# Soltanilara/av-aloha

Measured on AMD Instinct MI355X. Metric: env-steps/sec (whole node) at 4096 parallel envs, SlotInsertion-3Arms, higher is better.
Workload: dtype f32

## Files before the change

### av_aloha_amd/_ffi.py

```python
import ctypes as C
import os

import numpy as np

HERE = os.path.dirname(os.path.abspath(__file__))
LIB_PATH = os.path.join(HERE, "libavsim.so")

AVSIM_IO_DEVICE = 1
AVSIM_F64_PHYSICS = 2
IK_REFERENCE, IK_DLS = 0, 1
NDIMS = 12

_lib = None


class AvsimError(RuntimeError):
    pass


def lib():
    global _lib
    if _lib is None:
        if not os.path.exists(LIB_PATH):
            raise AvsimError(f"{LIB_PATH} is missing: build it with `python -m av_aloha_amd.build` "
                             "(there is no CPU fallback for the simulation path)")
        L = C.CDLL(LIB_PATH)
        vp, i32, u32, dbl = C.c_void_p, C.c_int, C.c_uint32, C.c_double
        L.avsim_create.argtypes = [vp, C.c_size_t, i32, i32, u32, C.POINTER(vp)]
        L.avsim_destroy.argtypes = [vp]
        L.avsim_destroy.restype = None
        L.avsim_last_error.argtypes = [vp]
        L.avsim_last_error.restype = C.c_char_p
        L.avsim_dims.argtypes = [vp, vp]
        L.avsim_set_option.argtypes = [vp, C.c_char_p, dbl]
        L.avsim_reset.argtypes = [vp, vp, vp]
        L.avsim_step.argtypes = [vp, vp, i32, vp, vp, vp]
        L.avsim_step_cartesian.argtypes = [vp, vp, i32, i32, vp, vp, vp]
        L.avsim_step_ctrl.argtypes = [vp, i32, vp, vp, vp]
        L.avsim_ik.argtypes = [vp, i32, i32, i32, i32, vp, vp, vp, vp]
        L.avsim_fk_jac.argtypes = [vp, i32, i32, vp, vp, vp]
        L.avsim_observe.argtypes = [vp, vp, vp, vp]
        L.avsim_set_qpos.argtypes = [vp, vp]
        L.avsim_get_state.argtypes = [vp, vp, vp, vp, vp]
        L.avsim_set_state.argtypes = [vp, vp, vp, vp, vp]
        L.avsim_get_reset_poses.argtypes = [vp, vp]
        L.avsim_set_reset_poses.argtypes = [vp, vp]
        L.avsim_get_latch.argtypes = [vp, vp]
        L.avsim_set_latch.argtypes = [vp, vp]
        L.avsim_get_contacts.argtypes = [vp, vp, vp, vp]
# ... 98 lines not shown
```

### av_aloha_amd/csrc/avsim_api.hip

```cpp
#include <hip/hip_runtime.h>

#include <cmath>
#include <cstdarg>
#include <cstdio>
#include <cstdlib>
#include <cstring>
#include <memory>
#include <string>
#include <vector>

#include "../../include/avsim.h"
#include "avsim_chunks.hip.h"
#include "avsim_compose.hip.h"
#include "avsim_imgprep.hip.h"
#include "avsim_obshist.hip.h"
#include "avsim_imgaug.hip.h"
#include "avsim_imgresize.hip.h"
#include "avsim_pointcloud.hip.h"
#include "avsim_episode.hip.h"
#include "avsim_ik.hip.h"
#include "avsim_io.h"
#include "avsim_jpeg.hip.h"
#include "avsim_model.h"
#include "avsim_phys.hip.h"
// ... 387 lines not shown
    if (!std::strcmp(name, "diffik_iters")) { h->ik.diff_iters = (int)value; return AVSIM_OK; }
    if (!std::strcmp(name, "gradik_iters")) { h->ik.grad_iters = (int)value; return AVSIM_OK; }
    try {
        if (h->phys.set_option(name, value)) {
            if (!std::strcmp(name, "num_joints")) h->nj = (int)value;
            return AVSIM_OK;
        }
    } catch (const std::exception& ex) {
        h->set_error("avsim_set_option(%s): %s", name, ex.what());
        return AVSIM_EHIP;
    }
    h->set_error("avsim_set_option: unknown option '%s'", name);
    return AVSIM_EINVAL;
}

int avsim_sync(avsim_t* h) {
    if (!h) return AVSIM_EINVAL;
    AVS_ON_DEVICE(h);
    HIPCHK(h, hipStreamSynchronize(h->stream));
    return AVSIM_OK;
}

int avsim_set_stream(avsim_t* h, void* s) {
    if (!h) return AVSIM_EINVAL;
    AVS_ON_DEVICE(h);
    HIPCHK(h, hipStreamSynchronize(h->stream));
    if (h->own_stream && h->stream) (void)hipStreamDestroy(h->stream);
    h->stream = (hipStream_t)s;
    h->own_stream = false;
    return AVSIM_OK;
// ... 1065 lines not shown
```

### av_aloha_amd/csrc/avsim_phys.hip.h

```cpp
#pragma once
#include <hip/hip_runtime.h>

#include <cstddef>
#include <cstring>
#include <string>
#include <type_traits>
#include <vector>

#include "avsim_collide.hip.h"
#include "avsim_dev.h"
#include "avsim_math.hip.h"
#include "avsim_model.h"
#include "avsim_phys_layout.h"

namespace avs {

enum { J_FREE = 0, J_BALL = 1, J_SLIDE = 2, J_HINGE = 3 };
enum { R_EQ = 0, R_FLOSS = 1, R_LIMIT = 2, R_CONTACT = 3 };
constexpr int TREE_W = 8;
constexpr int ROW_W = 2 * TREE_W;
constexpr int ROW_S = ROW_W;
constexpr int CAND_MAX = 256;
constexpr int PROF_W = 26;
constexpr int NEAR_MAX = 512;
// ... 116 lines not shown
    int hull_ovf;
    GLB_PTR(const int) pair_geom;
    GLB_PTR(const int) pair_condim;
    GLB_PTR(const real) pair_friction;
    GLB_PTR(const real) pair_solref;
    GLB_PTR(const real) pair_solimp;
    GLB_PTR(const real) pair_margin;
    GLB_PTR(const real) pair_gap;
    real* rJ_glob;
    real* rB_glob;
    real* gA_glob;
    int* near_glob;
    int* cand_glob;
    real* gref_glob;
    real* bxo_glob;
    GLB_PTR(const int) obs_qposadr;
    GLB_PTR(const real) obs_offset;
    GLB_PTR(const real) obs_scale;
};

template <typename real> using DevModel = DevModelT<real, DevHead<real>>;

static_assert(NARROW_SCR_W == 64 * SLOT_W + 4 * 56, "avsim_phys_layout.h: narrow-phase scratch");

template <typename real>
struct KArgs {
    DevModel<real> m;
    Layout lay;
    MOff mo;
};
template <typename real>
using KPtr = const KArgs<real> __attribute__((address_space(4)))*;

struct GenericSpec {};
template <typename SPEC> constexpr bool spec_fixed = !std::is_same<SPEC, GenericSpec>::value;
template <typename real, typename SPEC>
struct KFixed {
    using Model = DevModelT<real, FixedHead<real, SPEC>>;
    using FH = FixedHead<real, SPEC>;
    using DH = DevHead<real>;
    static_assert(sizeof(FH) == sizeof(DH) && alignof(FH) == alignof(DH) && sizeof(Model) == sizeof(DevModel<real>) && offsetof(FH, timestep) == offsetof(DH, timestep) &&
                      offsetof(FH, newton_tol) == offsetof(DH, newton_tol) && offsetof(FH, pad_tail_) == offsetof(DH, ls_iterations),
                  "FixedHead: the words of DevHead");
    KPtr<real> p;
    struct View {
        const Model __attribute__((address_space(4)))& m;
        static constexpr Layout lay = SPEC::lay;
        static constexpr MOff mo = SPEC::mo;
        AVS_DEV const View* operator->() const { return this; }
    };
// ... 7 lines not shown
template <typename real, typename SPEC> using KRef = typename KRefOf<real, SPEC>::type;
#define PHASE_LAUNDER()                                                                                \
    do {                                                                                               \
        const unsigned long long p_ = (unsigned long long)ka;                                          \
        unsigned lo_ = __builtin_amdgcn_readfirstlane((unsigned)p_), hi_ = __builtin_amdgcn_readfirstlane((unsigned)(p_ >> 32)); \
        asm volatile("" : "+s"(lo_), "+s"(hi_));                                                       \
        ka = (decltype(ka))(((unsigned long long)hi_ << 32) | lo_);                                    \
    } while (0)
#if defined(__HIP_DEVICE_COMPILE__)
#define AVS_ASSUME_LDS(p) __builtin_assume(__builtin_amdgcn_is_shared((const void*)(p)))
#else
#define AVS_ASSUME_LDS(p) ((void)(p))
#endif
template <typename T>
AVS_DEV T* lds_at(unsigned byte_off) { return (T*)(__attribute__((address_space(3))) T*)(size_t)byte_off; }
#define LDS_BASES()                                                                       \
    real* const r = this->r; AVS_ASSUME_LDS(r);     \
    int* const ii = this->ii; AVS_ASSUME_LDS(ii);   \
    (void)r; (void)ii
#define PHASE_BEGIN() PHASE_LAUNDER(); LDS_BASES()



#ifndef AVS_SYNC_SCOPE
#define AVS_SYNC_SCOPE "workgroup"
#endif
#define GSYNC()                                              \
    do {                                                     \
        __builtin_amdgcn_fence(__ATOMIC_ACQ_REL, AVS_SYNC_SCOPE); \
        __builtin_amdgcn_wave_barrier();                     \
    } while (0)
// ... 2080 lines not shown
                        const bool o = isbox && k >= BOX_SLOTC;
                        cdist[c] = o ? ov[4 * (k - BOX_SLOTC)] : scr[k];
                        cpair[c] = p;
                        for (int q = 0; q < 3; q++) { cpos[3 * c + q] = o ? ov[4 * (k - BOX_SLOTC) + 1 + q] : scr[SLOT_P + 3 * k + q]; cnrm[3 * c + q] = scr[SLOT_N + q]; }
                    }
                }
            if (ncon + tot > ka->lay.maxcon) ovf = 1;
            ncon = ncon + tot < ka->lay.maxcon ? ncon + tot : ka->lay.maxcon;
        }
        if (lane == 0) { misc[0] = ncon; misc[2] |= ovf; }
        GSYNC();
        t_narrow += __builtin_readcyclecounter() - tb1;
    }

#ifndef AVS_NO_SPLIT_PRE
    __device__ AVS_OUTLINE void pre_phases() {
        Env e(*this);
        e.kinematics(); e.crb(); e.rne_bias(); e.smooth();
    }
    __device__ AVS_OUTLINE void post_phases() {
        Env e(*this);
        e.euler(); e.check_divergence();
        diverged = e.diverged;
    }
#endif
    __device__ AVS_OUTLINE void make_constraints() {
        Env e(*this);
        e.make_constraints_i();
        diverged = e.diverged; nit_sum = e.nit_sum; nit_max = e.nit_max; t_broad = e.t_broad; t_narrow = e.t_narrow;
    }
    __device__ __attribute__((always_inline)) void make_constraints_i() {
        PHASE_BEGIN();
#ifdef AVSIM_PROBE_ROWS
        long long tpr_ = __builtin_readcyclecounter();
#define ROWPROBE(k) do { if (profiling) { const long long t_ = __builtin_readcyclecounter(); if (lane == 0) (ii + ka->lay.nprof)[8 + (k)] += (int)(t_ - tpr_); tpr_ = t_; } } while (0)
#else
#define ROWPROBE(k) ((void)0)
#endif
        real *qpos = r + ka->lay.qpos, *qvel = r + ka->lay.qvel;
        int *misc = ii + ka->lay.misc, *rmeta = ii + ka->lay.rmeta, *cpair = ii + ka->lay.cpair, *cefc = ii + ka->lay.cefc;
        real *cdist = r + ka->lay.cdist, *cpos = r + ka->lay.cpos, *cnrm = r + ka->lay.cnrm;
        int ncon = misc[0];
        int nefc = ka->m.neq + ka->m.nfloss;
        for (int i = lane; i < ka->m.neq; i += G) rmeta[i] = R_EQ | (i << 2);
        for (int i = lane; i < ka->m.nfloss; i += G) rmeta[ka->m.neq + i] = R_FLOSS | (i << 2);
        for (int base = 0; base < ka->m.nlimited; base += G) {
            int li = base + lane, lo = 0, hi = 0, j = 0;
            if (li < ka->m.nlimited) {
                j = limited_jnt_()[li];
                real q = qpos[jnt_qposadr_()[j]];
                lo = (q - jnt_range_()[2 * j]) < jnt_margin_()[j];
                hi = (jnt_range_()[2 * j + 1] - q) < jnt_margin_()[j];
            }
            int t1, t2, r1 = group_rank<G>(lo, grp, lane, &t1), r2 = group_rank<G>(hi, grp, lane, &t2);
            int pos = nefc + r1 + r2;
            if (lo && pos < ka->lay.maxefc) rmeta[pos] = R_LIMIT | (j << 2) | (0 << 12);
            if (hi && pos + lo < ka->lay.maxefc) rmeta[pos + lo] = R_LIMIT | (j << 2) | (1 << 12);
// ... 383 lines not shown
        PHASE_BEGIN();
        if constexpr (spec_fixed<SPEC>) { solver = ka->m.solver; newton_iters = ka->m.newton_iters; }
        int *misc = ii + ka->lay.misc, *rmeta = ii + ka->lay.rmeta, *cefc = ii + ka->lay.cefc, *rowI = ii + ka->lay.rowI;
        real *qacc = r + ka->lay.qacc, *as = r + ka->lay.asm_, *rowS = r + ka->lay.rowS, *fcon = r + ka->lay.fcon;
        GLB_PTR(real) rJ = rows_();
        int nefc = misc[1], ncon = misc[0];
        real* Minv = r + ka->lay.Minv;
        if (solver == 1) {
            real* warm = r + ka->lay.warm;
            for (int k = lane; k < ka->m.nv; k += G) qacc[k] = warm[k];
            GSYNC();
            bool two_ = false;
            for (int i = lane; i < nefc; i += G) two_ = two_ || ((rowI[i] >> 19) & 15) != 0;
            const bool coupled = __any(two_) != 0 || ka->m.ntree > 8;
#define AVS_NEWTON_ARGS ka, (GLB_PTR(const real))rJ, (LDS_PTR(real))r, (LDS_PTR(int))ii, (LDS_PTR(const int))LI(), nefc, ncon, misc[4], newton_iters, newton_tol, scale, profiling ? 1 : 0
            int used = __builtin_amdgcn_readfirstlane(ncon) <= 64 ? (coupled ? newton_solve_coupled<real, 1>(AVS_NEWTON_ARGS) : newton_solve<real, 1, false>(AVS_NEWTON_ARGS))
                                                                  : (coupled ? newton_solve_coupled<real, 2>(AVS_NEWTON_ARGS) : newton_solve<real, 2, false>(AVS_NEWTON_ARGS));
#undef AVS_NEWTON_ARGS
            nit_sum += used; nit_max = used > nit_max ? used : nit_max;
            GSYNC();
            long long tn0 = profiling ? __builtin_readcyclecounter() : 0;
            int done_ = 0;
            if (ka->m.noslip_trees && lead_per_tree() && __builtin_amdgcn_readfirstlane(misc[8]) == 0)
                done_ = noslip_trees<real>((LDS_PTR(real))rowS, (LDS_PTR(const int))rowI, (LDS_PTR(const int))cefc, (GLB_PTR(const real))rJ, (LDS_PTR(real))qacc,
                                           (LDS_PTR(const int))(ii + ka->lay.gI), (GLB_PTR(const real))coup_(), ncon, nefc, ka->m.noslip_iters, real(1e-6) / ka->m.nscale, NL_ARGS(noslip_lead()));
            if (__builtin_amdgcn_readfirstlane(done_) == 2)
                done_ = noslip_trees2<real>((LDS_PTR(real))rowS, (LDS_PTR(const int))rowI, (LDS_PTR(const int))cefc, (GLB_PTR(const real))rJ, (GLB_PTR(const real))rowsB_(), (LDS_PTR(real))qacc,
                                            (LDS_PTR(const int))(ii + ka->lay.gI), (GLB_PTR(const real))coup_(), ncon, nefc, ka->m.noslip_iters, real(1e-6) / ka->m.nscale, NL_ARGS(noslip_lead()));
            if (__builtin_amdgcn_readfirstlane(done_) != 1 && lane == 0) misc[8] = 1;
            if (__builtin_amdgcn_readfirstlane(done_) != 1)
            pgs_groups<real>((LDS_PTR(real))rowS, (LDS_PTR(const int))rowI, (GLB_PTR(const real))rJ, (GLB_PTR(const real))rowsB_(), (LDS_PTR(real))qacc,
// ... 130 lines not shown
#endif
__global__ void __launch_bounds__(64 * MAXW) AVSIM_PHYS_ATTR k_phys(KPtr<real> ka_small_, const real* __restrict__ img_real, const int* __restrict__ img_int, int N, int nsub, int pgs_iters, const float* __restrict__ action,
                                             int want_reward, real* __restrict__ g_qpos, real* __restrict__ g_qvel, real* __restrict__ g_ctrl,
                                             real* __restrict__ g_warm, int* __restrict__ g_latch, double* __restrict__ o_agent,
                                             int* __restrict__ o_reward, unsigned char* __restrict__ o_success, int* __restrict__ o_ncon,
                                             int* __restrict__ o_cpairs, double* __restrict__ o_cdist, int* __restrict__ o_diag, int max_reward, int export_contacts, long long* __restrict__ o_prof, float* __restrict__ o_xpose,
                                             const int* __restrict__ env_order, int* __restrict__ o_cost, int* __restrict__ work_head, int* __restrict__ work_next,
                                             int* __restrict__ retry, int retry_mode, KPtr<real> ka_big_) {
    const KRef<real, SPEC> ka_small(ka_small_), ka_big(ka_big_);
    extern __shared__ __attribute__((aligned(16))) unsigned char smem[];
    int nwork = N;
    const bool pass2 = RETRY && ((retry_mode & 7) == 2 || (retry_mode & 7) == 4);
    const bool pass1 = RETRY && ((retry_mode & 7) == 1 || (retry_mode & 7) == 3);
    if (pass2) {
        nwork = retry[(retry_mode & 7) == 4];
        if (blockIdx.x == 0 && threadIdx.x == 0) { *work_next = 0; retry[(retry_mode & 7) == 2] = 0; }
        if (nwork <= 0) return;
    }
    int* const bigflag = retry + 2 + N;
    const int cap1_con = pass2 ? (retry_mode >> 8) & 0x3ff : ka_small->lay.maxcon, cap1_efc = pass2 ? (retry_mode >> 18) & 0x3ff : ka_small->lay.maxefc;
    int* const pair_want = reinterpret_cast<int*>(smem + (size_t)(blockDim.x >> 6) * ka_small->lay.bytes_per_env + (size_t)ka_small->mo.nreal * sizeof(real) + (size_t)ka_small->mo.nint * 4);
    int* const pair_grant = pair_want + MAXW / 2;
    if (RETRY && threadIdx.x < MAXW / 2) { pair_want[threadIdx.x] = 0; pair_grant[threadIdx.x] = 0; }
    static_assert(G == 64, "one env per wavefront");
#ifdef AVSIM_NO_PROF
    o_prof = nullptr;
#endif
    const int wpb = blockDim.x >> 6;
    const int wave = threadIdx.x >> 6, lane = threadIdx.x & 63, grp = 0;
    constexpr bool FIXED = spec_fixed<SPEC>;
    static_assert(!(FIXED && RETRY), "the per-model kernels are one-pass");
    size_t rec0 = 0;
    if constexpr (FIXED) {
        rec0 = (((size_t)ka_small->mo.nreal * sizeof(real) + (size_t)ka_small->mo.nint * 4) + 15) & ~(size_t)15;
        if ((unsigned)(size_t)(LDS_PTR(unsigned char))smem != 0u) return;
    }
    real* lr = reinterpret_cast<real*>(smem + (FIXED ? (size_t)0 : (size_t)wpb * ka_small->lay.bytes_per_env));
    int* li = reinterpret_cast<int*>(lr + ka_small->mo.nreal);
    for (int i = threadIdx.x; i < ka_small->mo.nreal; i += blockDim.x) lr[i] = img_real[i];
    for (int i = threadIdx.x; i < ka_small->mo.nint; i += blockDim.x) li[i] = img_int[i];
    if (blockIdx.x == 0 && threadIdx.x == 0) *work_next = 0;
    __syncthreads();
    const int pr = wave >> 1;
    const bool paired = pass1 && (retry_mode & 8) && (wave | 1) < wpb;
    auto lds_get = [&](int* p) { int v = 0; if (lane == 0) v = __hip_atomic_load(p, __ATOMIC_ACQUIRE, __HIP_MEMORY_SCOPE_WORKGROUP); return __builtin_amdgcn_readfirstlane(v); };
    auto lds_put = [&](int* p, int v) { if (lane == 0) __hip_atomic_store(p, v, __ATOMIC_RELEASE, __HIP_MEMORY_SCOPE_WORKGROUP); };
    auto to_list = [&](int e) { if (lane == 0) retry[2 + atomicAdd(retry + ((retry_mode & 7) == 3), 1)] = e; };
    constexpr int PAIR_LEFT = -1;
    int claim_gen = 0, my_claim = 0;
    auto park = [&]() {
        for (;;) {
            const int w = lds_get(&pair_want[pr]);
            if (w == 0 || (w & 0xff) == wave + 1) break;
            lds_put(&pair_grant[pr], w);
            __builtin_amdgcn_s_sleep(32);
        }
// ... 41 lines not shown
    KRef<real, SPEC> ka = (RETRY && big) ? ka_big : ka_small;
    const long long t_launch = __builtin_readcyclecounter();
    real* r = reinterpret_cast<real*>(smem + rec0 + (size_t)((RETRY && big) ? (wave & ~1) : wave) * ka_small->lay.bytes_per_env);
    int* ii = reinterpret_cast<int*>(r + ka->lay.nreal);
    bool beyond = false;
    Env<real, G, SPEC> E(ka, r, ii, lane, grp, lr, li);
    E.env = env;

    for (int i = lane; i < ka->m.nq; i += G) r[ka->lay.qpos + i] = g_qpos[(size_t)env * ka->m.nq + i];
    for (int i = lane; i < ka->m.nv; i += G) { r[ka->lay.qvel + i] = g_qvel[(size_t)env * ka->m.nv + i]; r[ka->lay.warm + i] = g_warm[(size_t)env * ka->m.nv + i]; }
    for (int i = lane; i < ka->m.nu; i += G) r[ka->lay.ctrl + i] = g_ctrl[(size_t)env * ka->m.nu + i];
    if (lane == 0) for (int k = 0; k < 8; k++) { ii[ka->lay.misc + k] = 0; ii[ka->lay.nprof + k] = 0; ii[ka->lay.nprof + 8 + k] = 0; }
    if (lane == 0) ii[ka->lay.misc + 8] = 0;
    E.profiling = o_prof != nullptr;
    GSYNC();
    if (action) {
        const float* a = action + (size_t)env * ka->m.nj;
        for (int i = lane; i < ka->m.nj; i += G) {
            real v = (real)a[i];
            if (i == 6 || i == 13) v = v * (ka->m.grip_hi - ka->m.grip_lo) + ka->m.grip_lo;
            r[ka->lay.ctrl + i] = v;
        }
        GSYNC();
    }
    long long tp[9] = {0, 0, 0, 0, 0, 0, 0, 0, 0};
#define PROF(k, stmt) do { if (o_prof) { long long t0_ = __builtin_readcyclecounter(); stmt; tp[k] += __builtin_readcyclecounter() - t0_; } else { stmt; } } while (0)
    for (int s = 0; s < nsub; s++) {
#ifndef AVS_NO_SPLIT_PRE
        PROF(0, E.pre_phases());
#else
        {
            Env<real, G, SPEC> e(E);
            PROF(0, e.kinematics());
            PROF(1, e.crb());
            PROF(2, e.rne_bias());
            PROF(3, e.smooth());
        }
#endif
        PROF(4, E.collide());
        PROF(5, E.make_constraints());
        if (RETRY) beyond = beyond || ii[ka->lay.misc + 0] > cap1_con || ii[ka->lay.misc + 1] > cap1_efc;
        PROF(6, E.solve(pgs_iters, ka->m.solver, ka->m.newton_iters, ka->m.newton_tol, ka->m.nscale));
#ifndef AVS_NO_SPLIT_PRE
        PROF(7, E.post_phases());
#else
        {
            Env<real, G, SPEC> e(E);
            PROF(7, e.euler());
            e.check_divergence();
            E.diverged = e.diverged;
        }
#endif
    }
    if (o_prof && lane == 0) {
        for (int k = 0; k < 8; k++) o_prof[(size_t)env * PROF_W + k] = tp[k];
        o_prof[(size_t)env * PROF_W + 8] = E.t_broad; o_prof[(size_t)env * PROF_W + 9] = E.t_narrow;
        for (int k = 0; k < 16; k++) o_prof[(size_t)env * PROF_W + 10 + k] = ii[ka->lay.nprof + k];
    }
    int nefc_last = ii[ka->lay.misc + 1];
    E.kinematics();
    if (o_xpose) {
        for (int b = lane; b < ka->m.nbody; b += G) {
            float* o = o_xpose + ((size_t)env * ka->m.nbody + b) * 12;
            for (int k = 0; k < 3; k++) o[k] = (float)r[ka->lay.xpos + 3 * b + k];
            for (int k = 0; k < 9; k++) o[3 + k] = (float)r[ka->lay.xmat + 9 * b + k];
        }
    }
    E.collide();
    if (RETRY && pass1 && !big && (ii[ka->lay.misc + 2] & 3)) {
        if (paired) redo_env = env; else to_list(env);
        GSYNC();
        continue;
    }
    if (RETRY) {
        beyond = beyond || ii[ka->lay.misc + 0] > cap1_con;
        if (lane == 0 && (big || pass2 || (retry_mode & 8))) bigflag[env] = beyond ? 1 : 0;
    }

    if (nsub > 0) {
        for (int i = lane; i < ka->m.nq; i += G) g_qpos[(size_t)env * ka->m.nq + i] = r[ka->lay.qpos + i];
        for (int i = lane; i < ka->m.nv; i += G) { g_qvel[(size_t)env * ka->m.nv + i] = r[ka->lay.qvel + i]; g_warm[(size_t)env * ka->m.nv + i] = r[ka->lay.warm + i]; }
    }
    if (action) for (int i = lane; i < ka->m.nu; i += G) g_ctrl[(size_t)env * ka->m.nu + i] = r[ka->lay.ctrl + i];
    if (o_agent)
        for (int i = lane; i < ka->m.nj; i += G) o_agent[(size_t)env * ka->m.nj + i] = ((double)r[ka->lay.qpos + ka->m.obs_qposadr[i]] - (double)ka->m.obs_offset[i]) * (double)ka->m.obs_scale[i];
    int ncon = ii[ka->lay.misc + 0];
    if (want_reward) {
        int latch = g_latch[env];
        int rw = E.reward(&latch);
        if (lane == 0) {
            g_latch[env] = latch;
// ... 13 lines not shown
    }
    if (lane == 0 && o_cost && nsub > 0) o_cost[env] = (int)((__builtin_readcyclecounter() - t_launch) >> 6);
    if (lane == 0 && !o_xpose) {
        o_ncon[env] = ncon;
        bool bad = E.diverged != 0;
        for (int i = 0; i < ka->m.nq; i++) bad |= !(fabs(r[ka->lay.qpos + i]) < real(1e6));
        o_diag[4 * env] = ncon; o_diag[4 * env + 1] = nefc_last; o_diag[4 * env + 2] = ii[ka->lay.misc + 2]; o_diag[4 * env + 3] = (bad ? 1 : 0) | ((ii[ka->lay.misc + 3] & 0xff) << 8) | ((E.nit_sum & 0xfff) << 16) | ((E.nit_max < 15 ? E.nit_max : 15) << 28);
    }
    GSYNC();
    if (RETRY && big && pass1) {
        lds_put(&pair_want[pr], 0);
    }
  }
    if (RETRY && paired) lds_put(&pair_grant[pr], PAIR_LEFT);
}

static __global__ void __launch_bounds__(1024) k_env_order(const int* __restrict__ cost, int* __restrict__ order, int N) {
    __shared__ int lo, hi, cnt[256], off[256];
    if (threadIdx.x == 0) { lo = 0x7fffffff; hi = 0; }
    if (threadIdx.x < 256) cnt[threadIdx.x] = 0;
    __syncthreads();
    int mn = 0x7fffffff, mx = 0;
    for (int i = threadIdx.x; i < N; i += 1024) { const int c = cost[i]; mn = c < mn ? c : mn; mx = c > mx ? c : mx; }
    atomicMin(&lo, mn);
    atomicMax(&hi, mx);
    __syncthreads();
    const int base = lo;
    const float scale = 255.0f / (float)(hi - lo + 1);
    auto bucket = [&](int c) { const int b = 255 - (int)((float)(c - base) * scale); return b < 0 ? 0 : (b > 255 ? 255 : b); };
    for (int i = threadIdx.x; i < N; i += 1024) atomicAdd(&cnt[bucket(cost[i])], 1);
// ... 310 lines not shown
        if (rows.alloc((size_t)N * maxefc * ROW_S * (f64 ? 8 : 4) * 2) != hipSuccess) throw std::runtime_error("hipMalloc of the constraint row buffers failed");
        mf.rJ_glob = rows.as<float>(); md.rJ_glob = rows.as<double>();
        mf.rB_glob = mf.rJ_glob + (size_t)N * maxefc * ROW_S; md.rB_glob = md.rJ_glob + (size_t)N * maxefc * ROW_S;
        if (gref.alloc(((size_t)N * dims[4] * 3 + (size_t)N * 64 * BOX_OVF_W) * (f64 ? 8 : 4)) != hipSuccess) throw std::runtime_error("hipMalloc of the Verlet reference buffer failed");
        mf.gref_glob = gref.as<float>(); md.gref_glob = gref.as<double>();
        mf.bxo_glob = mf.gref_glob + (size_t)N * dims[4] * 3; md.bxo_glob = md.gref_glob + (size_t)N * dims[4] * 3;
        if (coup.alloc((size_t)N * lay2.maxgrp * GA_W * (f64 ? 8 : 4)) != hipSuccess || near.alloc((size_t)N * (NEAR_MAX + CAND_MAX) * 4) != hipSuccess)
            throw std::runtime_error("hipMalloc of the coupling / neighbour buffers failed");
        int* const d_near = near.as<int>();
        mf.gA_glob = coup.as<float>(); md.gA_glob = coup.as<double>(); mf.near_glob = d_near; md.near_glob = d_near; mf.cand_glob = md.cand_glob = d_near + (size_t)N * NEAR_MAX;
        kargs_dirty = true;
        if (cpairs.alloc((size_t)N * maxcon * 8) != hipSuccess || cdist.alloc((size_t)N * maxcon * 8) != hipSuccess)
            throw std::runtime_error("hipMalloc of the contact export buffers failed");
        (void)hipMemset(cpairs.ptr(), 0xff, (size_t)N * maxcon * 8);
        (void)hipMemset(cdist.ptr(), 0, (size_t)N * maxcon * 8);
    }
    bool init(const Blob& b, int N_, bool f64_, std::string& err) {
        N = N_;
        f64 = f64_;
        try {
            if (f64) build(b, md); else build(b, mf);
            static const int mx[5] = {4, 4, 5, 3, 4};
            max_reward = mx[b.scalar("task_id")];
            int ms = f64 ? md.msize : mf.msize;
            const int *cap_efc = CAP_EFC, *cap_con = CAP_CON, *cap_efc1 = CAP_EFC1, *cap_con1 = CAP_CON1;
            maxefc = cap_efc[b.scalar("task_id")];
            maxcon = cap_con[b.scalar("task_id")];
            maxefc1 = cap_efc1[b.scalar("task_id")];
            maxcon1 = cap_con1[b.scalar("task_id")];
            dims[0] = b.scalar("nq"); dims[1] = b.scalar("nv"); dims[2] = b.scalar("nu"); dims[3] = b.scalar("nbody"); dims[4] = b.scalar("ngeom"); dims[5] = ms; dims[6] = b.scalar("ntree");
            make_layout(dims[0], dims[1], dims[2], dims[3], dims[4], dims[5], dims[6]);
            d_qpos_home = up(b.f("qpos_home"));
            d_ctrl_home = up(b.f("ctrl_home"));
            d_obj_qadr = up(b.i("objects_qposadr"));
            d_ncon = up(std::vector<int>((size_t)N, 0));
            d_diag = up(std::vector<int>((size_t)N * 4, 0));
            d_cost = up(std::vector<int>((size_t)N, 0));
            d_order = up(std::vector<int>((size_t)N, 0));
            d_retry = up(std::vector<int>(2 * (size_t)N + 2, 0));
            alloc_contacts();
        } catch (const std::exception& e) {
            err = std::string("physics init: ") + e.what();
            return false;
        }
        return true;
    }
    bool set_option(const char* name, double v) {
        std::string n(name);
        kargs_dirty = true;
        if (n == "pgs_iters") { pgs_iters = (int)v; return true; }
        if (n == "solver") { if (v != 0 && v != 1) return false; mf.solver = md.solver = (int)v; return true; }
        if (n == "newton_iters") { if (v < 1 || v > 100) return false; mf.newton_iters = md.newton_iters = (int)v; return true; }
        if (n == "newton_tol") { if (v < 0) return false; mf.newton_tol = (float)v; md.newton_tol = v; return true; }
        if (n == "ls_tolerance") { if (!(v > 0) || v >= 1) return false; mf.ls_tolerance = (float)v; md.ls_tolerance = v; return true; }
        if (n == "ls_iterations") { if (v < 1 || v > 1000) return false; mf.ls_iterations = md.ls_iterations = (int)v; return true; }
        if (n == "export_contacts") { export_contacts = v != 0; return true; }
        if (n == "num_joints") { if (v != 14 && v != 21) return false; mf.nj = md.nj = (int)v; return true; }
        if (n == "order_envs") { order_envs = v != 0; return true; }
        if (n == "phys_specialised") { if (v != 0 && v != 1 && v != 2) return false; specialised = (int)v; return true; }
        if (n == "pair_waves") { pair_waves = v != 0; return true; }
        if (n == "qcqp_tridiag") { mf.qcqp_tridiag = md.qcqp_tridiag = v < 0 ? 0 : (v > 2 ? 2 : (int)v); return true; }
        if (n == "noslip_iters") { if (v < 0 || v > 100) return false; mf.noslip_iters = md.noslip_iters = (int)v; return true; }
        if (n == "noslip_per_tree") { mf.noslip_per_tree = md.noslip_per_tree = v != 0; return true; }
        if (n == "noslip_trees") { mf.noslip_trees = md.noslip_trees = v != 0; return true; }
        if (n == "newton_component") { mf.newton_component = md.newton_component = v != 0; return true; }
        if (n == "newton_early_exit") { mf.newton_early_exit = md.newton_early_exit = v != 0; return true; }
        if (n == "persist_blocks") { int x = (int)v; if (x >= 1 && x <= 64) { persist_over = x; return true; } return false; }
        if (n == "waves_per_block") { int x = (int)v; if (x >= 0 && x <= AVSIM_PHYS_MAXW) { wpb_override = x; return true; } return false; }
        if (n == "profile_phases") {
            if (v != 0 && !d_prof) d_prof = up(std::vector<long long>((size_t)N * PROF_W, 0));
            if (v == 0) d_prof = nullptr;
            return true;
        }
        if (n == "maxefc" || n == "maxcon" || n == "maxefc_first" || n == "maxcon_first") {
            int x = (int)v;
// ... 5 lines not shown
            alloc_contacts();
            return true;
        }
        return false;
    }

    template <typename real, int MAXW>
    int waves_per_block(const Layout& L) const {
        const size_t tables = (size_t)moff.nreal * sizeof(real) + (size_t)moff.nint * 4;
        int wpb = tables < 160 * 1024 ? (int)((160 * 1024 - tables) / (size_t)L.bytes_per_env) : 0;
        if (wpb > MAXW) wpb = MAXW;
        if (wpb_override > 0) wpb = wpb_override < MAXW ? wpb_override : MAXW;
        return wpb < 1 ? 1 : wpb;
    }

    template <typename real, int G, int MAXW>
    int launch_t(hipStream_t st, const DevModel<real>& m, int nsub, const float* action, void* qpos, void* qvel, void* ctrl, void* warm,
                 int* latch, double* agent, int32_t* reward, uint8_t* success, std::string& err) {
        const size_t tables = (size_t)moff.nreal * sizeof(real) + (size_t)moff.nint * 4;
        auto kern1 = k_phys<real, G, MAXW, false>;
        auto kern2 = k_phys<real, G, MAXW, true>;
        const char* spec_name = nullptr;
        const void* kspec = sizeof(real) == 4 && MAXW == AVSIM_PHYS_MAXW ? spec_kernel(&spec_name) : nullptr;
        if (refuses(err)) return -1;
        if (spec_note != (kspec ? 1 : 2) && getenv("AVSIM_DEBUG_LAYOUT")) {
            fprintf(stderr, "avsim: k_phys %s%s\n", kspec ? "specialised for " : "generic", kspec ? spec_name : "");
            spec_note = kspec ? 1 : 2;
        }
        if (!attr_done) {
            hipError_t e = hipFuncSetAttribute((const void*)kern1, hipFuncAttributeMaxDynamicSharedMemorySize, 160 * 1024);
            if (e == hipSuccess) e = hipFuncSetAttribute((const void*)kern2, hipFuncAttributeMaxDynamicSharedMemorySize, 160 * 1024);
            if (e != hipSuccess) { err = std::string("hipFuncSetAttribute: ") + hipGetErrorString(e); return -3; }
            int dev = 0;
            hipDeviceProp_t prop;
            if (hipGetDevice(&dev) == hipSuccess && hipGetDeviceProperties(&prop, dev) == hipSuccess && prop.multiProcessorCount > 0) num_cu = prop.multiProcessorCount;
            if (!head) {
                if (head.reserve(2 * sizeof(int)) != hipSuccess) { err = "hipMalloc(work counters) failed"; return -3; }
                (void)hipMemset(head.ptr(), 0, 2 * sizeof(int));
            }
            attr_done = 1;
        }
        if (kspec) {
            if (!(attr_done & 2)) {
                const hipError_t e = hipFuncSetAttribute(kspec, hipFuncAttributeMaxDynamicSharedMemorySize, 160 * 1024);
                if (e != hipSuccess) { err = std::string("hipFuncSetAttribute(") + spec_name + "): " + hipGetErrorString(e); return -3; }
                attr_done |= 2;
            }
            kern1 = (decltype(kern1))kspec;
        }
        const bool two = two_pass();
        int wpb = waves_per_block<real, MAXW>(lay);
        const int wpb2 = waves_per_block<real, MAXW>(lay2);
        if (!two && wpb_override <= 0 && num_cu > 0 && N < num_cu * wpb) { wpb = (N + num_cu - 1) / num_cu; if (wpb < 1) wpb = 1; }
        const size_t pairflags = two ? 2 * (MAXW / 2 > 0 ? MAXW / 2 : 1) * sizeof(int) : 0;
        const size_t shmem = (size_t)lay.bytes_per_env * wpb + tables + pairflags, shmem2 = (size_t)lay2.bytes_per_env * wpb2 + tables + pairflags;
        const int pairing = (two && wpb >= 2 && lay2.bytes_per_env <= 2 * lay.bytes_per_env && pair_waves) ? 8 : 0;
        if (shmem > 160 * 1024 || (two && shmem2 > 160 * 1024)) { err = "per-block LDS exceeds 160 KiB; lower maxefc/maxcon"; return -1; }
        const int per_cu = (int)((160 * 1024) / shmem) > 0 ? (int)((160 * 1024) / shmem) : 1;
        int nblk = num_cu * per_cu * (persist_over > 0 ? persist_over : 1);
        if (nblk > (N + wpb - 1) / wpb) nblk = (N + wpb - 1) / wpb;
        if (kargs_dirty) {
            KArgs<real> ka{m, lay, moff}, ka2{m, lay2, moff};
            if (kargs.reserve(sizeof(KArgs<double>)) != hipSuccess || kargs2.reserve(sizeof(KArgs<double>)) != hipSuccess) { err = "hipMalloc(kernel arguments) failed"; return -3; }
            (void)hipStreamSynchronize(st);
            if (hipMemcpy(kargs.ptr(), &ka, sizeof(ka), hipMemcpyHostToDevice) != hipSuccess || hipMemcpy(kargs2.ptr(), &ka2, sizeof(ka2), hipMemcpyHostToDevice) != hipSuccess) { err = "hipMemcpy(kernel arguments) failed"; return -3; }
            kargs_dirty = false;
        }
        static_assert((8 | 7) < (1 << 8), "retry_mode: mode bits and pairing flag below bit 8");
        if (two && (maxcon1 >= 1024 || maxefc1 >= 1024 || maxcon1 < 0 || maxefc1 < 0)) { err = "first-tier capacities do not fit the 10-bit fields of retry_mode (maxcon_first / maxefc_first < 1024)"; return -1; }
        const int* order = nullptr;
        if (order_envs && have_cost && nsub > 0 && N > wpb) {
            hipLaunchKernelGGL(k_env_order, dim3(1), dim3(1024), 0, st, (const int*)d_cost, d_order, N);
            order = d_order;
        }
        const int want_reward = (reward || success) && (nsub > 0 || force_reward) ? 1 : 0;
        const int par = (int)(retry_parity & 1);
        int* const rlist = d_retry + 2;
// ... 55 lines not shown
```

### av_aloha_amd/sim.py

```python
import ctypes as C
import json
import os

import numpy as np

from . import _ffi, images
from .constants import MODEL_DIR, SIM_PHYSICS_ENV_STEP_RATIO

TASK_KEYS = ("insert_peg", "slot_insertion", "sew_needle", "tube_transfer", "hook_package")


VARIANT_PREFIX = {"gym": "", "data_collection": "dc_"}


def load_blob(task, num_arms, variant="gym"):
    base = os.path.join(MODEL_DIR, f"{VARIANT_PREFIX[variant]}{task}_{num_arms}arms")
    with open(base + ".avm", "rb") as f:
        blob = f.read()
    with open(base + ".json") as f:
        manifest = json.load(f)
    return blob, manifest


class BatchedSim(images.ImageCalls):
# ... 5 lines not shown
        blob = file_blob if blob is None else blob
        self.h = _ffi.Handle(blob, num_envs, device, _ffi.AVSIM_F64_PHYSICS if f64 else 0)
        self.N = num_envs
        self._jpeg_stride = {}
        for k in ("nq", "nv", "nu", "nj", "nobj", "max_reward", "maxcon", "maxefc"):
            setattr(self, k, getattr(self.h, k))
        for k, v in (options or {}).items():
            self.set_option(k, v)

    def set_option(self, name, value):
        self.h.check(self.h.L.avsim_set_option(self.h.h, name.encode(), float(value)))
        if name in ("maxcon", "maxefc"):
            d = np.zeros(_ffi.NDIMS, dtype=np.int32)
            self.h.check(self.h.L.avsim_dims(self.h.h, d.ctypes.data))
            self.maxcon, self.maxefc = int(d[8]), int(d[9])

    def reset(self, obj_qpos, mask=None):
        obj = np.ascontiguousarray(obj_qpos, dtype=np.float64).reshape(self.N, self.nobj * 7)
        m = None if mask is None else np.ascontiguousarray(mask, dtype=np.uint8)
        self.h.check(self.h.L.avsim_reset(self.h.h, _ffi.ptr(m), obj.ctypes.data))

    def step(self, action, nsub=SIM_PHYSICS_ENV_STEP_RATIO, want_reward=True):
        a = np.ascontiguousarray(action, dtype=np.float32).reshape(self.N, self.nj)
        ap = np.empty((self.N, self.nj))
        rw = np.empty(self.N, dtype=np.int32) if want_reward else None
        su = np.empty(self.N, dtype=np.uint8) if want_reward else None
        self.h.check(self.h.L.avsim_step(self.h.h, a.ctypes.data, nsub, ap.ctypes.data, _ffi.ptr(rw), _ffi.ptr(su)))
        return ap, rw, (su.astype(bool) if su is not None else None)

    def step_ctrl(self, nsub=SIM_PHYSICS_ENV_STEP_RATIO):
# ... 277 lines not shown
```

### include/avsim.h

```cpp
#ifndef AVSIM_H
#define AVSIM_H
#include <stddef.h>
#include <stdint.h>

#ifdef __cplusplus
extern "C" {
#endif

typedef struct avsim avsim_t;

enum {
    AVSIM_OK = 0,
    AVSIM_EINVAL = -1,
    AVSIM_ENODEV = -2,
    AVSIM_EHIP = -3,
    AVSIM_EMODEL = -4,
    AVSIM_ENOTIMPL = -5
};

enum {
    AVSIM_IO_DEVICE = 1u << 0,
    AVSIM_F64_PHYSICS = 1u << 1
};

enum {
    AVSIM_IK_REFERENCE = 0,
    AVSIM_IK_DLS = 1
};

#define AVSIM_NDIMS 12

int avsim_create(const void* model_blob, size_t nbytes, int num_envs, int device, uint32_t flags, avsim_t** out);
void avsim_destroy(avsim_t* h);
const char* avsim_last_error(const avsim_t* h);
int avsim_dims(const avsim_t* h, int32_t dims[AVSIM_NDIMS]);

int avsim_set_option(avsim_t* h, const char* name, double value);

int avsim_reset(avsim_t* h, const uint8_t* mask, const double* obj_qpos);

int avsim_step(avsim_t* h, const float* action, int nsub, double* agent_pos, int32_t* reward, uint8_t* success);

int avsim_step_ctrl(avsim_t* h, int nsub, double* agent_pos, int32_t* reward, uint8_t* success);

int avsim_step_cartesian(avsim_t* h, const double* action23, int ik_mode, int nsub, double* agent_pos,
                         int32_t* reward, uint8_t* success);

int avsim_ik(avsim_t* h, int arm, int controller, int max_iters, int n, const double* q, const double* pos,
             const double* quat_wxyz, double* q_out);
int avsim_fk_jac(avsim_t* h, int arm, int n, const double* q, double* T, double* J);

int avsim_observe(avsim_t* h, double* agent_pos, int32_t* reward, uint8_t* success);
// ... 119 lines not shown
```

Measured before the change: 1.046 million.

## Carry end-of-step kinematics and contacts into next step's first substep

```diff
diff --git a/av_aloha_amd/_ffi.py b/av_aloha_amd/_ffi.py
--- a/av_aloha_amd/_ffi.py
+++ b/av_aloha_amd/_ffi.py
@@ -33,6 +33,7 @@
         L.avsim_last_error.restype = C.c_char_p
         L.avsim_dims.argtypes = [vp, vp]
         L.avsim_set_option.argtypes = [vp, C.c_char_p, dbl]
+        L.avsim_get_option.argtypes = [vp, C.c_char_p, C.POINTER(dbl)]
         L.avsim_reset.argtypes = [vp, vp, vp]
         L.avsim_step.argtypes = [vp, vp, i32, vp, vp, vp]
         L.avsim_step_cartesian.argtypes = [vp, vp, i32, i32, vp, vp, vp]
diff --git a/av_aloha_amd/csrc/avsim_api.hip b/av_aloha_amd/csrc/avsim_api.hip
--- a/av_aloha_amd/csrc/avsim_api.hip
+++ b/av_aloha_amd/csrc/avsim_api.hip
@@ -425,6 +425,21 @@
     return AVSIM_EINVAL;
 }
 
+int avsim_get_option(avsim_t* h, const char* name, double* value) {
+    if (!h || !name || !value) return AVSIM_EINVAL;
+    AVS_ON_DEVICE(h);
+    if (!std::strcmp(name, "phys_carry")) { *value = h->phys.carry; return AVSIM_OK; }
+    if (!std::strcmp(name, "phys_wave_slots")) { *value = h->phys.wave_slots(); return AVSIM_OK; }
+    if (!std::strcmp(name, "phys_carry_hits")) {
+        int hits = 0;
+        if (h->phys.carry_hits(h->stream, &hits)) { h->set_error("avsim_get_option(phys_carry_hits): reading the counter failed"); return AVSIM_EHIP; }
+        *value = hits;
+        return AVSIM_OK;
+    }
+    h->set_error("avsim_get_option: unknown option '%s'", name);
+    return AVSIM_EINVAL;
+}
+
 int avsim_sync(avsim_t* h) {
     if (!h) return AVSIM_EINVAL;
     AVS_ON_DEVICE(h);
diff --git a/av_aloha_amd/csrc/avsim_phys.hip.h b/av_aloha_amd/csrc/avsim_phys.hip.h
--- a/av_aloha_amd/csrc/avsim_phys.hip.h
+++ b/av_aloha_amd/csrc/avsim_phys.hip.h
@@ -154,6 +154,10 @@
     int* cand_glob;
     real* gref_glob;
     real* bxo_glob;
+    real* carry_r;
+    int* carry_i;
+    int carry_gen;
+    int carry_on;
     GLB_PTR(const int) obs_qposadr;
     GLB_PTR(const real) obs_offset;
     GLB_PTR(const real) obs_scale;
@@ -174,6 +178,8 @@
 
 struct GenericSpec {};
 template <typename SPEC> constexpr bool spec_fixed = !std::is_same<SPEC, GenericSpec>::value;
+template <typename SPEC, bool FIXED = spec_fixed<SPEC>> struct SpecOneConPerLane : std::false_type {};
+template <typename SPEC> struct SpecOneConPerLane<SPEC, true> : std::integral_constant<bool, (SPEC::maxcon <= 64)> {};
 template <typename real, typename SPEC>
 struct KFixed {
     using Model = DevModelT<real, FixedHead<real, SPEC>>;
@@ -211,7 +217,9 @@
 #endif
 template <typename T>
 AVS_DEV T* lds_at(unsigned byte_off) { return (T*)(__attribute__((address_space(3))) T*)(size_t)byte_off; }
-#define LDS_BASES()                                                                       \
+AVS_DEV unsigned real_bits(float x) { return __builtin_bit_cast(unsigned, x); }
+AVS_DEV unsigned long long real_bits(double x) { return __builtin_bit_cast(unsigned long long, x); }
+#define LDS_BASES()                                                                   \
     real* const r = this->r; AVS_ASSUME_LDS(r);     \
     int* const ii = this->ii; AVS_ASSUME_LDS(ii);   \
     (void)r; (void)ii
@@ -2322,9 +2330,10 @@
     }
 
 #ifndef AVS_NO_SPLIT_PRE
-    __device__ AVS_OUTLINE void pre_phases() {
+    __device__ AVS_OUTLINE void pre_phases(bool have_kin) {
         Env e(*this);
-        e.kinematics(); e.crb(); e.rne_bias(); e.smooth();
+        if (!have_kin) e.kinematics();
+        e.crb(); e.rne_bias(); e.smooth();
     }
     __device__ AVS_OUTLINE void post_phases() {
         Env e(*this);
@@ -2349,6 +2358,7 @@
         int *misc = ii + ka->lay.misc, *rmeta = ii + ka->lay.rmeta, *cpair = ii + ka->lay.cpair, *cefc = ii + ka->lay.cefc;
         real *cdist = r + ka->lay.cdist, *cpos = r + ka->lay.cpos, *cnrm = r + ka->lay.cnrm;
         int ncon = misc[0];
+        if constexpr (spec_fixed<SPEC>) { constexpr int cap_con = SPEC::maxcon; __builtin_assume(ncon >= 0 && ncon <= cap_con); }
         int nefc = ka->m.neq + ka->m.nfloss;
         for (int i = lane; i < ka->m.neq; i += G) rmeta[i] = R_EQ | (i << 2);
         for (int i = lane; i < ka->m.nfloss; i += G) rmeta[ka->m.neq + i] = R_FLOSS | (i << 2);
@@ -2762,7 +2772,11 @@
             for (int i = lane; i < nefc; i += G) two_ = two_ || ((rowI[i] >> 19) & 15) != 0;
             const bool coupled = __any(two_) != 0 || ka->m.ntree > 8;
 #define AVS_NEWTON_ARGS ka, (GLB_PTR(const real))rJ, (LDS_PTR(real))r, (LDS_PTR(int))ii, (LDS_PTR(const int))LI(), nefc, ncon, misc[4], newton_iters, newton_tol, scale, profiling ? 1 : 0
-            int used = __builtin_amdgcn_readfirstlane(ncon) <= 64 ? (coupled ? newton_solve_coupled<real, 1>(AVS_NEWTON_ARGS) : newton_solve<real, 1, false>(AVS_NEWTON_ARGS))
+            int used;
+            if constexpr (SpecOneConPerLane<SPEC>::value)
+                used = coupled ? newton_solve_coupled<real, 1>(AVS_NEWTON_ARGS) : newton_solve<real, 1, false>(AVS_NEWTON_ARGS);
+            else
+                used = __builtin_amdgcn_readfirstlane(ncon) <= 64 ? (coupled ? newton_solve_coupled<real, 1>(AVS_NEWTON_ARGS) : newton_solve<real, 1, false>(AVS_NEWTON_ARGS))
                                                                   : (coupled ? newton_solve_coupled<real, 2>(AVS_NEWTON_ARGS) : newton_solve<real, 2, false>(AVS_NEWTON_ARGS));
 #undef AVS_NEWTON_ARGS
             nit_sum += used; nit_max = used > nit_max ? used : nit_max;
@@ -2923,7 +2937,7 @@
     const bool pass1 = RETRY && ((retry_mode & 7) == 1 || (retry_mode & 7) == 3);
     if (pass2) {
         nwork = retry[(retry_mode & 7) == 4];
-        if (blockIdx.x == 0 && threadIdx.x == 0) { *work_next = 0; retry[(retry_mode & 7) == 2] = 0; }
+        if (blockIdx.x == 0 && threadIdx.x == 0) { *work_next = 0; work_next[2] = 0; retry[(retry_mode & 7) == 2] = 0; }
         if (nwork <= 0) return;
     }
     int* const bigflag = retry + 2 + N;
@@ -2948,7 +2962,7 @@
     int* li = reinterpret_cast<int*>(lr + ka_small->mo.nreal);
     for (int i = threadIdx.x; i < ka_small->mo.nreal; i += blockDim.x) lr[i] = img_real[i];
     for (int i = threadIdx.x; i < ka_small->mo.nint; i += blockDim.x) li[i] = img_int[i];
-    if (blockIdx.x == 0 && threadIdx.x == 0) *work_next = 0;
+    if (blockIdx.x == 0 && threadIdx.x == 0) { *work_next = 0; work_next[2] = 0; }
     __syncthreads();
     const int pr = wave >> 1;
     const bool paired = pass1 && (retry_mode & 8) && (wave | 1) < wpb;
@@ -3020,6 +3034,21 @@
     if (lane == 0) ii[ka->lay.misc + 8] = 0;
     E.profiling = o_prof != nullptr;
     GSYNC();
+#define AVS_CARRY_PTRS()                                                                                                                        \
+    const int carry_nkin = ka->lay.M - ka->lay.xpos, carry_rw = ka->m.nq + carry_nkin + 7 * ka->lay.expcon, carry_iw = 8 + ka->lay.expcon;         \
+    int cenv_ = __builtin_amdgcn_readfirstlane(env);                                                                                            \
+    asm volatile("" : "+s"(cenv_));                                                                                                             \
+    GLB_PTR(real) const cr = (GLB_PTR(real))ka->m.carry_r + (size_t)cenv_ * carry_rw;                                                           \
+    GLB_PTR(int) const ci = (GLB_PTR(int))ka->m.carry_i + (size_t)cenv_ * carry_iw;                                                             \
+    (void)carry_nkin; (void)cr; (void)ci
+    bool carried = false;
+    if (!RETRY && ka->m.carry_on != 0 && nsub > 0) {
+        AVS_CARRY_PTRS();
+        bool same = ci[0] == ka->m.carry_gen;
+        for (int i = lane; i < ka->m.nq; i += G) same = same && real_bits(cr[i]) == real_bits(r[ka->lay.qpos + i]);
+        carried = __builtin_amdgcn_readfirstlane(__any(!same)) == 0;
+        if (carried && lane == 0) atomicAdd(work_head + 2, 1);
+    }
     if (action) {
         const float* a = action + (size_t)env * ka->m.nj;
         for (int i = lane; i < ka->m.nj; i += G) {
@@ -3032,17 +3061,36 @@
     long long tp[9] = {0, 0, 0, 0, 0, 0, 0, 0, 0};
 #define PROF(k, stmt) do { if (o_prof) { long long t0_ = __builtin_readcyclecounter(); stmt; tp[k] += __builtin_readcyclecounter() - t0_; } else { stmt; } } while (0)
     for (int s = 0; s < nsub; s++) {
+        const bool from_carry = carried && s == 0;
+        if (from_carry) {
+            AVS_CARRY_PTRS();
+            for (int i = lane; i < carry_nkin; i += G) r[ka->lay.xpos + i] = cr[ka->m.nq + i];
+            GSYNC();
+        }
 #ifndef AVS_NO_SPLIT_PRE
-        PROF(0, E.pre_phases());
+        PROF(0, E.pre_phases(from_carry));
 #else
         {
             Env<real, G, SPEC> e(E);
-            PROF(0, e.kinematics());
+            if (!from_carry) PROF(0, e.kinematics());
             PROF(1, e.crb());
             PROF(2, e.rne_bias());
             PROF(3, e.smooth());
         }
 #endif
+        if (from_carry) {
+            AVS_CARRY_PTRS();
+            int nc = __builtin_amdgcn_readfirstlane(ci[1]);
+            nc = nc < 0 ? 0 : (nc < ka->lay.maxcon ? nc : ka->lay.maxcon);
+            GLB_PTR(const real) cc = cr + ka->m.nq + carry_nkin;
+            for (int c = lane; c < nc; c += G) { r[ka->lay.cdist + c] = cc[c]; ii[ka->lay.cpair + c] = ci[8 + c]; }
+            for (int i = lane; i < 3 * nc; i += G) { r[ka->lay.cpos + i] = cc[ka->lay.expcon + i]; r[ka->lay.cnrm + i] = cc[4 * ka->lay.expcon + i]; }
+            if (lane == 0) {
+                ii[ka->lay.misc + 0] = nc; ii[ka->lay.misc + 3] = ci[2]; ii[ka->lay.misc + 2] |= ci[3];
+                ii[ka->lay.misc + 6] = ci[4]; ii[ka->lay.misc + 7] = ci[5];
+            }
+            GSYNC();
+        } else
         PROF(4, E.collide());
         PROF(5, E.make_constraints());
         if (RETRY) beyond = beyond || ii[ka->lay.misc + 0] > cap1_con || ii[ka->lay.misc + 1] > cap1_efc;
@@ -3072,7 +3120,28 @@
             for (int k = 0; k < 9; k++) o[3 + k] = (float)r[ka->lay.xmat + 9 * b + k];
         }
     }
+    int flags_sub = 0;
+    const bool carry_write = !RETRY && ka->m.carry_on != 0;
+    if (carry_write) {
+        flags_sub = __builtin_amdgcn_readfirstlane(ii[ka->lay.misc + 2]);
+        if (lane == 0) ii[ka->lay.misc + 2] = 0;
+    }
     E.collide();
+    if (carry_write) {
+        AVS_CARRY_PTRS();
+        const int flags_col = ii[ka->lay.misc + 2], nc = ii[ka->lay.misc + 0];
+        GLB_PTR(real) cc = cr + ka->m.nq + carry_nkin;
+        for (int i = lane; i < ka->m.nq; i += G) cr[i] = r[ka->lay.qpos + i];
+        for (int i = lane; i < carry_nkin; i += G) cr[ka->m.nq + i] = r[ka->lay.xpos + i];
+        for (int c = lane; c < nc; c += G) { cc[c] = r[ka->lay.cdist + c]; ci[8 + c] = ii[ka->lay.cpair + c]; }
+        for (int i = lane; i < 3 * nc; i += G) { cc[ka->lay.expcon + i] = r[ka->lay.cpos + i]; cc[4 * ka->lay.expcon + i] = r[ka->lay.cnrm + i]; }
+        if (lane == 0) {
+            ci[0] = ka->m.carry_gen; ci[1] = nc; ci[2] = ii[ka->lay.misc + 3]; ci[3] = flags_col;
+            ci[4] = ii[ka->lay.misc + 6]; ci[5] = ii[ka->lay.misc + 7];
+            ii[ka->lay.misc + 2] = flags_sub | flags_col;
+        }
+        GSYNC();
+    }
     if (RETRY && pass1 && !big && (ii[ka->lay.misc + 2] & 3)) {
         if (paired) redo_env = env; else to_list(env);
         GSYNC();
@@ -3081,6 +3150,7 @@
     if (RETRY) {
         beyond = beyond || ii[ka->lay.misc + 0] > cap1_con;
         if (lane == 0 && (big || pass2 || (retry_mode & 8))) bigflag[env] = beyond ? 1 : 0;
+        if (lane == 0 && ka->m.carry_i) ((GLB_PTR(int))ka->m.carry_i)[(size_t)env * (8 + ka->lay.expcon)] = 0;
     }
 
     if (nsub > 0) {
@@ -3124,6 +3194,7 @@
   }
     if (RETRY && paired) lds_put(&pair_grant[pr], PAIR_LEFT);
 }
+#undef AVS_CARRY_PTRS
 
 static __global__ void __launch_bounds__(1024) k_env_order(const int* __restrict__ cost, int* __restrict__ order, int N) {
     __shared__ int lo, hi, cnt[256], off[256];
@@ -3464,6 +3535,22 @@
             throw std::runtime_error("hipMalloc of the contact export buffers failed");
         (void)hipMemset(cpairs.ptr(), 0xff, (size_t)N * maxcon * 8);
         (void)hipMemset(cdist.ptr(), 0, (size_t)N * maxcon * 8);
+        const size_t rb = (size_t)N * carry_rw() * (f64 ? 8 : 4), ib = (size_t)N * carry_iw() * 4;
+        if (carrybuf.alloc(rb + ib) != hipSuccess) throw std::runtime_error("hipMalloc of the carry records failed");
+        (void)hipMemset(carrybuf.ptr(), 0, rb + ib);
+        mf.carry_r = carrybuf.as<float>(); md.carry_r = carrybuf.as<double>();
+        mf.carry_i = md.carry_i = reinterpret_cast<int*>(carrybuf.as<char>() + rb);
+    }
+    int carry = 1;
+    unsigned carry_gen = 0;
+    DevBuf carrybuf;
+    int carry_rw() const { return dims[0] + (lay2.M - lay2.xpos) + 7 * lay2.expcon; }
+    int carry_iw() const { return 8 + lay2.expcon; }
+    int carry_hits(hipStream_t st, int* hits) {
+        *hits = 0;
+        if (!head || launch_count == 0) return 0;
+        if (hipStreamSynchronize(st) != hipSuccess) return -3;
+        return hipMemcpy(hits, head.as<int>() + 2 + ((launch_count - 1) & 1), sizeof(int), hipMemcpyDeviceToHost) == hipSuccess ? 0 : -3;
     }
     bool init(const Blob& b, int N_, bool f64_, std::string& err) {
         N = N_;
@@ -3488,6 +3575,8 @@
             d_cost = up(std::vector<int>((size_t)N, 0));
             d_order = up(std::vector<int>((size_t)N, 0));
             d_retry = up(std::vector<int>(2 * (size_t)N + 2, 0));
+            mf.carry_r = nullptr; md.carry_r = nullptr; mf.carry_i = md.carry_i = nullptr;
+            mf.carry_gen = md.carry_gen = 0; mf.carry_on = md.carry_on = 0;
             alloc_contacts();
         } catch (const std::exception& e) {
             err = std::string("physics init: ") + e.what();
@@ -3509,6 +3598,7 @@
         if (n == "order_envs") { order_envs = v != 0; return true; }
         if (n == "phys_specialised") { if (v != 0 && v != 1 && v != 2) return false; specialised = (int)v; return true; }
         if (n == "pair_waves") { pair_waves = v != 0; return true; }
+        if (n == "phys_carry") { if (v != 0 && v != 1) return false; carry = (int)v; return true; }
         if (n == "qcqp_tridiag") { mf.qcqp_tridiag = md.qcqp_tridiag = v < 0 ? 0 : (v > 2 ? 2 : (int)v); return true; }
         if (n == "noslip_iters") { if (v < 0 || v > 100) return false; mf.noslip_iters = md.noslip_iters = (int)v; return true; }
         if (n == "noslip_per_tree") { mf.noslip_per_tree = md.noslip_per_tree = v != 0; return true; }
@@ -3544,6 +3634,14 @@
         return wpb < 1 ? 1 : wpb;
     }
 
+    int wave_slots() const {
+        const size_t tables = (size_t)moff.nreal * (f64 ? 8 : 4) + (size_t)moff.nint * 4;
+        const int wpb = f64 ? waves_per_block<double, 4>(lay) : waves_per_block<float, AVSIM_PHYS_MAXW>(lay);
+        const size_t shmem = (size_t)lay.bytes_per_env * wpb + tables;
+        const int per_cu = (int)((160 * 1024) / shmem) > 0 ? (int)((160 * 1024) / shmem) : 1;
+        return num_cu * per_cu * wpb;
+    }
+
     template <typename real, int G, int MAXW>
     int launch_t(hipStream_t st, const DevModel<real>& m, int nsub, const float* action, void* qpos, void* qvel, void* ctrl, void* warm,
                  int* latch, double* agent, int32_t* reward, uint8_t* success, std::string& err) {
@@ -3565,8 +3663,8 @@
             hipDeviceProp_t prop;
             if (hipGetDevice(&dev) == hipSuccess && hipGetDeviceProperties(&prop, dev) == hipSuccess && prop.multiProcessorCount > 0) num_cu = prop.multiProcessorCount;
             if (!head) {
-                if (head.reserve(2 * sizeof(int)) != hipSuccess) { err = "hipMalloc(work counters) failed"; return -3; }
-                (void)hipMemset(head.ptr(), 0, 2 * sizeof(int));
+                if (head.reserve(4 * sizeof(int)) != hipSuccess) { err = "hipMalloc(work counters) failed"; return -3; }
+                (void)hipMemset(head.ptr(), 0, 4 * sizeof(int));
             }
             attr_done = 1;
         }
@@ -3591,6 +3689,9 @@
         if (nblk > (N + wpb - 1) / wpb) nblk = (N + wpb - 1) / wpb;
         if (kargs_dirty) {
             KArgs<real> ka{m, lay, moff}, ka2{m, lay2, moff};
+            if (++carry_gen == 0) carry_gen = 1;
+            ka.m.carry_gen = ka2.m.carry_gen = (int)carry_gen;
+            ka.m.carry_on = ka2.m.carry_on = carry;
             if (kargs.reserve(sizeof(KArgs<double>)) != hipSuccess || kargs2.reserve(sizeof(KArgs<double>)) != hipSuccess) { err = "hipMalloc(kernel arguments) failed"; return -3; }
             (void)hipStreamSynchronize(st);
             if (hipMemcpy(kargs.ptr(), &ka, sizeof(ka), hipMemcpyHostToDevice) != hipSuccess || hipMemcpy(kargs2.ptr(), &ka2, sizeof(ka2), hipMemcpyHostToDevice) != hipSuccess) { err = "hipMemcpy(kernel arguments) failed"; return -3; }
diff --git a/av_aloha_amd/sim.py b/av_aloha_amd/sim.py
--- a/av_aloha_amd/sim.py
+++ b/av_aloha_amd/sim.py
@@ -43,6 +43,11 @@
             d = np.zeros(_ffi.NDIMS, dtype=np.int32)
             self.h.check(self.h.L.avsim_dims(self.h.h, d.ctypes.data))
             self.maxcon, self.maxefc = int(d[8]), int(d[9])
+
+    def get_option(self, name):
+        v = C.c_double(0.0)
+        self.h.check(self.h.L.avsim_get_option(self.h.h, name.encode(), C.byref(v)))
+        return v.value
 
     def reset(self, obj_qpos, mask=None):
         obj = np.ascontiguousarray(obj_qpos, dtype=np.float64).reshape(self.N, self.nobj * 7)
diff --git a/include/avsim.h b/include/avsim.h
--- a/include/avsim.h
+++ b/include/avsim.h
@@ -36,6 +36,7 @@
 int avsim_dims(const avsim_t* h, int32_t dims[AVSIM_NDIMS]);
 
 int avsim_set_option(avsim_t* h, const char* name, double value);
+int avsim_get_option(avsim_t* h, const char* name, double* value);
 
 int avsim_reset(avsim_t* h, const uint8_t* mask, const double* obj_qpos);
 
```

Result: no change. 1.053 million, median of 6 (+0.7%).
